# ukrbublik/You-Can-Not-Recommend

Hardware: AMD Instinct MI355X
Metric: ALS ratings/sec per iteration (U+I solve) (higher is better)
Workload: dtype f32

## Files before the change

you-can-not-recommend_amd/csrc/als_kernels.hip.h:

```cpp
#pragma once
#include <hip/hip_runtime.h>
#include <type_traits>
#include <stdint.h>
#include "schedule.h"

#ifndef YCNR_FUSED_WAVES_PER_SIMD
#define YCNR_FUSED_WAVES_PER_SIMD 2
#endif
#ifndef YCNR_FUSED_PREFETCH
#define YCNR_FUSED_PREFETCH 2
#endif

#ifndef YCNR_DUAL_BATCH
#define YCNR_DUAL_BATCH true
#endif
#ifndef YCNR_SLAB_PREFETCH
#define YCNR_SLAB_PREFETCH 3
#endif
#ifndef YCNR_DPP_PIVOTS
#define YCNR_DPP_PIVOTS 1
#endif
#ifndef YCNR_EDGE4_SOLVE
#define YCNR_EDGE4_SOLVE 1
#endif
// ... 2376 lines not shown
  const bool remF32 = krem == 4 || krem == 8;
  const int ksteps32 = remF32 ? (k >> 5) : ((k + 31) >> 5);
  const int first = 4 * (int)blockIdx.x;
  Unit us[4];
#pragma unroll
  for (int s = 0; s < 4; ++s) us[s] = a.units[a.firstDual + min(first + s, count - 1)];
  int ns[4];
#pragma unroll
  for (int s = 0; s < 4; ++s) ns[s] = (int)(us[s].end - us[s].beg);
  const int nmax = max(max(ns[0], ns[1]), max(ns[2], ns[3]));
  const int n_g = g == 0 ? ns[0] : g == 1 ? ns[1] : g == 2 ? ns[2] : ns[3];
  const int64_t beg_g = g == 0 ? us[0].beg : g == 1 ? us[1].beg : g == 2 ? us[2].beg : us[3].beg;
  const int row_g = g == 0 ? us[0].row : g == 1 ? us[1].row : g == 2 ? us[2].row : us[3].row;
  const bool valid_g = first + g < count;
  const int64_t q_g = beg_g + (c < n_g ? c : n_g - 1);
  const unsigned id_g = (unsigned)a.indx[q_g];
  float y = c < n_g ? a.vals[q_g] : 0.0f;
  acc_t acc[4];
#pragma unroll
  for (int s = 0; s < 4; ++s) {
    const int64_t q = us[s].beg + (c < ns[s] ? c : ns[s] - 1);
    const float *rowp = c < ns[s] ? a.fixed + (int64_t)a.indx[q] * k : a.zeros;
    float4 z[KS][2];
#pragma unroll
    for (int kk = 0; kk < KS; ++kk) {
      const int f = 32 * kk + 8 * g;
      z[kk][0] = *reinterpret_cast<const float4 *>(f < k ? rowp + f : a.zeros);
      z[kk][1] = *reinterpret_cast<const float4 *>(f + 4 < k ? rowp + f + 4 : a.zeros);
    }
    acc_t t = acc_t{0.0f, 0.0f, 0.0f, 0.0f};
    if (remF32) {
      const float y0 = rowp[(k & ~31) + g];
      t = Tr::mma(y0, y0, t);
      if (krem == 8) {
        const float y1 = rowp[(k & ~31) + 4 + g];
        t = Tr::mma(y1, y1, t);
      }
    }
#pragma unroll
    for (int kk = 0; kk < KS; ++kk) {
      if (kk < ksteps32) {
        const float x[8] = {z[kk][0].x, z[kk][0].y, z[kk][0].z, z[kk][0].w, z[kk][1].x, z[kk][1].y, z[kk][1].z, z[kk][1].w};
        unsigned h[4], m[4], l[4];
#pragma unroll
        for (int jj = 0; jj < 4; ++jj) {
          const float x0 = x[2 * jj], x1 = x[2 * jj + 1];
          const unsigned u0 = __builtin_bit_cast(unsigned, x0), u1 = __builtin_bit_cast(unsigned, x1);
          h[jj] = __builtin_amdgcn_perm(u1, u0, 0x07060302);
          const float s0 = x0 - __builtin_bit_cast(float, u0 & 0xFFFF0000u);
          const float s1 = x1 - __builtin_bit_cast(float, u1 & 0xFFFF0000u);
          const unsigned v0 = __builtin_bit_cast(unsigned, s0), v1 = __builtin_bit_cast(unsigned, s1);
          m[jj] = __builtin_amdgcn_perm(v1, v0, 0x07060302);
          const float t0 = s0 - __builtin_bit_cast(float, v0 & 0xFFFF0000u);
          const float t1 = s1 - __builtin_bit_cast(float, v1 & 0xFFFF0000u);
          l[jj] = __builtin_amdgcn_perm(__builtin_bit_cast(unsigned, t1), __builtin_bit_cast(unsigned, t0), 0x07060302);
        }
        const bf16x8 p1 = __builtin_bit_cast(bf16x8, u32x4{h[0], h[1], h[2], h[3]});
        const bf16x8 p2 = __builtin_bit_cast(bf16x8, u32x4{m[0], m[1], m[2], m[3]});
        const bf16x8 p3 = __builtin_bit_cast(bf16x8, u32x4{l[0], l[1], l[2], l[3]});
        t = __builtin_amdgcn_mfma_f32_16x16x32_bf16(p2, p2, t, 0, 0, 0);
        t = __builtin_amdgcn_mfma_f32_16x16x32_bf16(p1, p3, t, 0, 0, 0);
        t = __builtin_amdgcn_mfma_f32_16x16x32_bf16(p3, p1, t, 0, 0, 0);
        t = __builtin_amdgcn_mfma_f32_16x16x32_bf16(p1, p2, t, 0, 0, 0);
        t = __builtin_amdgcn_mfma_f32_16x16x32_bf16(p2, p1, t, 0, 0, 0);
        t = __builtin_amdgcn_mfma_f32_16x16x32_bf16(p1, p1, t, 0, 0, 0);
      }
    }
    acc[s] = t;
  }
  float R[16];
#pragma unroll
  for (int t = 0; t < 4; ++t) {
    const acc_t in = acc_t{acc[0][t], acc[1][t], acc[2][t], acc[3][t]};
    float out[4];
    Sv::transpose_rg(in, out);
#pragma unroll
    for (int q = 0; q < 4; ++q) R[4 * q + t] = out[q];
  }
  {
    const float dv = c < n_g ? (float)(a.lambda * (double)n_g) : 1.0f;
#pragma unroll
    for (int m = 0; m < 16; ++m) R[m] += c == m ? dv : 0.0f;
  }
  float myinv = 1.0f;
  bool bad = false;
  auto bc = [](float v, auto P) { return Sv::template row_bcast<decltype(P)::value>(v); };
  auto pivot = [&](auto P) {
    constexpr int p = decltype(P)::value;
    const float d = bc(R[p], P);
    bad = bad || !(d > 0.0f);
    const float inv = __builtin_amdgcn_rcpf(d);
    const float m = c > p ? R[p] * inv : 0.0f;
    myinv = c == p ? inv : myinv;
    auto upd = [&](auto J) {
      constexpr int j = decltype(J)::value;
      if constexpr (j > p) R[j] = fmaf(-m, bc(R[j], P), R[j]);
    };
    upd(std::integral_constant<int, 1>{}); upd(std::integral_constant<int, 2>{}); upd(std::integral_constant<int, 3>{});
    upd(std::integral_constant<int, 4>{}); upd(std::integral_constant<int, 5>{}); upd(std::integral_constant<int, 6>{});
    upd(std::integral_constant<int, 7>{}); upd(std::integral_constant<int, 8>{}); upd(std::integral_constant<int, 9>{});
    upd(std::integral_constant<int, 10>{}); upd(std::integral_constant<int, 11>{}); upd(std::integral_constant<int, 12>{});
    upd(std::integral_constant<int, 13>{}); upd(std::integral_constant<int, 14>{}); upd(std::integral_constant<int, 15>{});
    y = fmaf(-m, bc(y, P), y);
  };
#define YCNR_P(N) pivot(std::integral_constant<int, N>{});
  YCNR_P(0) YCNR_P(1) YCNR_P(2) YCNR_P(3) YCNR_P(4) YCNR_P(5) YCNR_P(6) YCNR_P(7)
  YCNR_P(8) YCNR_P(9) YCNR_P(10) YCNR_P(11) YCNR_P(12) YCNR_P(13) YCNR_P(14) YCNR_P(15)
#undef YCNR_P
  float w = 0.0f;
  auto back = [&](auto J) {
    constexpr int j = decltype(J)::value;
    const float t = y * myinv;
    w = c == j ? t : w;
    y = fmaf(-R[j], bc(t, J), y);
  };
#define YCNR_B(N) back(std::integral_constant<int, N>{});
  YCNR_B(15) YCNR_B(14) YCNR_B(13) YCNR_B(12) YCNR_B(11) YCNR_B(10) YCNR_B(9) YCNR_B(8)
  YCNR_B(7) YCNR_B(6) YCNR_B(5) YCNR_B(4) YCNR_B(3) YCNR_B(2) YCNR_B(1) YCNR_B(0)
#undef YCNR_B
  const char *base = reinterpret_cast<const char *>(a.fixed);
  const unsigned off0 = (unsigned)min(c, kq - 1) * 16u, off1 = (unsigned)min(c + 16, kq - 1) * 16u;
  float4 x0 = float4{0.0f, 0.0f, 0.0f, 0.0f}, x1 = float4{0.0f, 0.0f, 0.0f, 0.0f};
  auto gather = [&](auto I) {
    constexpr int i = decltype(I)::value;
    if (i < nmax) {
      const unsigned idi = __builtin_bit_cast(unsigned, bc(__builtin_bit_cast(float, id_g), I));
      const float wi = bc(w, I);
      const unsigned ro = idi * (unsigned)(k * 4);
      const float4 v0 = *reinterpret_cast<const float4 *>(base + (ro + off0));
      const float4 v1 = *reinterpret_cast<const float4 *>(base + (ro + off1));
      x0.x = fmaf(v0.x, wi, x0.x); x0.y = fmaf(v0.y, wi, x0.y); x0.z = fmaf(v0.z, wi, x0.z); x0.w = fmaf(v0.w, wi, x0.w);
      x1.x = fmaf(v1.x, wi, x1.x); x1.y = fmaf(v1.y, wi, x1.y); x1.z = fmaf(v1.z, wi, x1.z); x1.w = fmaf(v1.w, wi, x1.w);
    }
  };
#define YCNR_G(N) gather(std::integral_constant<int, N>{});
  YCNR_G(0) YCNR_G(1) YCNR_G(2) YCNR_G(3) YCNR_G(4) YCNR_G(5) YCNR_G(6) YCNR_G(7)
  YCNR_G(8) YCNR_G(9) YCNR_G(10) YCNR_G(11) YCNR_G(12) YCNR_G(13) YCNR_G(14) YCNR_G(15)
#undef YCNR_G
  if (valid_g) {
    float *out = a.solved + (int64_t)row_g * k;
    if (c < kq) *reinterpret_cast<float4 *>(out + 4 * c) = x0;
    if (c + 16 < kq) *reinterpret_cast<float4 *>(out + 4 * (c + 16)) = x1;
  }
  {
    const float chk = (x0.x + x0.y + x0.z + x0.w + x1.x + x1.y + x1.z + x1.w) * 0.0f;
    const unsigned long long m = __ballot(valid_g && (bad || !(chk == 0.0f)));
    if (c == 0 && ((m >> (16 * g)) & 0xFFFFull)) {
      atomicAdd(&a.err->count, 1);
      a.err->firstRow = row_g;
    }
  }
}

template <typename T, int NB, bool LDS_SOLVER, bool E4, bool FEW>
constexpr int reduce_waves() {
  if (!FEW || sizeof(T) != 4 || LDS_SOLVER) return 1;
  return NB <= 6 ? 3 : NB == 7 ? (E4 ? 3 : 2) : 1;
}
template <typename T, int NB, bool LDS_SOLVER, bool EDGE, bool E4 = false, bool FEW = false>
__global__ __launch_bounds__(64, (reduce_waves<T, NB, LDS_SOLVER, E4, FEW>())) void als_reduce_solve_kernel(StepArgs<T> a) {
  extern __shared__ __attribute__((aligned(16))) unsigned char smem[];
  using G = typename GramSel<T, NB, EDGE>::type;
  using acc_t = typename G::acc_t;
  const int lane = threadIdx.x;
  const SplitRow sr = a.split[blockIdx.x];
  typename G::State st;
  G::init(st);
  bool wide = false;
  if constexpr (std::is_same<T, float>::value && !FEW) wide = sr.nslabs > kFewSlabs;
  if (wide) {
    if constexpr (std::is_same<T, float>::value && !FEW)
      G::sum_slabs_wide(st, a.slabs + (int64_t)sr.slab0 * (G::slab_regs() * 64) + lane, sr.nslabs);
  } else {
    for (int sl = 0; sl < sr.nslabs; ++sl) G::add_slab(st, a.slabs + (int64_t)(sr.slab0 + sl) * (G::slab_regs() * 64) + lane);
  }
  acc_t acc[G::NT];
  T bacc[NB];
  G::to_tiles(st, acc, bacc, reinterpret_cast<T *>(smem), lane);
  const T lam = (T)(a.lambda * (double)sr.n);
  if constexpr (E4 && std::is_same<T, float>::value && !LDS_SOLVER) {
    SolveMfmaF32<NB>::template run<true>(acc, bacc, reinterpret_cast<float *>(smem), a.k, lam, a.solved + (int64_t)sr.row * a.k, sr.row, a.err, lane,
                                         a.kReal > 0 ? a.kReal : -1);
  } else {
    SolverFor<T, NB, LDS_SOLVER>::type::run(acc, bacc, reinterpret_cast<T *>(smem), a.k, lam,
                                          a.solved + (int64_t)sr.row * a.k, sr.row, a.err, lane, a.kReal > 0 ? a.kReal : -1);
  }
}


template <typename T>
__global__ __launch_bounds__(256) void als_slab_sum_kernel(T *arena, const SlabSum *list, int64_t elems) {
  const SlabSum e = list[blockIdx.x];
  for (int64_t i = threadIdx.x; i < elems; i += 256) {
    const T *src = arena + e.src0 + i;
    if (std::is_same<T, float>::value && e.n > kFewSlabs) {
      double v = 0.0;
      for (int s = 0; s < e.n; ++s) v += (double)src[(int64_t)s * elems];
      arena[e.dst + i] = (T)v;
    } else {
      T v = T(0);
      for (int s = 0; s < e.n; ++s) v += src[(int64_t)s * elems];
      arena[e.dst + i] = v;
    }
  }
}

template <typename T, int NB, bool LDS_SOLVER, bool EDGE, bool E4 = false>
__global__ __launch_bounds__(64, 1) void als_band_reduce_solve_kernel(StepArgs<T> a, const T *const *bandSlab, int32_t nBands) {
  extern __shared__ __attribute__((aligned(16))) unsigned char smem[];
  using G = typename GramSel<T, NB, EDGE>::type;
  using acc_t = typename G::acc_t;
  const int lane = threadIdx.x;
  const SplitRow sr = a.split[blockIdx.x];
  typename G::State st;
  G::init(st);
  for (int b = 0; b < nBands; ++b) {
    const T *p = bandSlab[(int64_t)sr.slab0 + b];
    if (p) G::add_slab(st, p + lane);
  }
  acc_t acc[G::NT];
  T bacc[NB];
  G::to_tiles(st, acc, bacc, reinterpret_cast<T *>(smem), lane);
  const T lam = (T)(a.lambda * (double)sr.n);
  if constexpr (E4 && std::is_same<T, float>::value && !LDS_SOLVER) {
    SolveMfmaF32<NB>::template run<true>(acc, bacc, reinterpret_cast<float *>(smem), a.k, lam, a.solved + (int64_t)sr.row * a.k, sr.row, a.err, lane,
                                         a.kReal > 0 ? a.kReal : -1);
  } else {
    SolverFor<T, NB, LDS_SOLVER>::type::run(acc, bacc, reinterpret_cast<T *>(smem), a.k, lam,
                                          a.solved + (int64_t)sr.row * a.k, sr.row, a.err, lane, a.kReal > 0 ? a.kReal : -1);
  }
}

template <typename T>
struct RmseArgs {
  const int64_t *rowPtr;
  const int32_t *indx;
  const T *vals;
  const T *userFactors;
  const T *itemFactors;
  const int64_t *portionRowEnd;
  double *out;
  double shift;
  int64_t rowBegin;
  int32_t k;
};

#ifndef YCNR_RMSE_RB
#define YCNR_RMSE_RB 4
#endif
template <typename T, int NCH>
__global__ __launch_bounds__(256) void als_rmse_kernel(RmseArgs<T> a) {
  __shared__ double red[3][16];
  const int tid = threadIdx.x, grp = tid >> 4, l16 = tid & 15;
  const int p = blockIdx.x;
  const int64_t r0 = p == 0 ? 0 : a.portionRowEnd[p - 1];
  const int64_t r1 = a.portionRowEnd[p];
  double sd2 = 0, sp = 0, cnt = 0;
  typedef T vec4 __attribute__((ext_vector_type(4)));
  constexpr int NC = NCH > 0 ? NCH : 1;
  constexpr int RB = NCH == 0 ? 1 : (NCH * (int)sizeof(T) <= 8 ? YCNR_RMSE_RB : (NCH * (int)sizeof(T) <= 16 ? YCNR_RMSE_RB / 2 : YCNR_RMSE_RB / 4));
  const int nchunk = a.k >> 2;
  for (int64_t r = r0 + grp; r < r1; r += 16) {
    const T *uF = a.userFactors + (a.rowBegin + r) * a.k;
    vec4 u[NC];
    if constexpr (NCH > 0) {
#pragma unroll
      for (int i = 0; i < NCH; ++i) {
        const int ch = l16 + 16 * i;
        u[i] = ch < nchunk ? *reinterpret_cast<const vec4 *>(uF + 4 * ch) : vec4{T(0), T(0), T(0), T(0)};
      }
    }
    const int64_t q1 = a.rowPtr[r + 1];
    for (int64_t q = a.rowPtr[r]; q < q1; q += RB) {
      int32_t id[RB];
      T val[RB];
#pragma unroll
      for (int j = 0; j < RB; ++j) {
        const int64_t qq = q + j < q1 ? q + j : q1 - 1;
        id[j] = a.indx[qq];
        val[j] = a.vals[qq];
      }
      vec4 v[RB][NC];
      if constexpr (NCH > 0) {
#pragma unroll
        for (int j = 0; j < RB; ++j) {
          const T *iF = a.itemFactors + (int64_t)id[j] * a.k;
#pragma unroll
          for (int i = 0; i < NCH; ++i) {
            const int ch = l16 + 16 * i;
            v[j][i] = ch < nchunk ? *reinterpret_cast<const vec4 *>(iF + 4 * ch) : vec4{T(0), T(0), T(0), T(0)};
          }
        }
      }
#pragma unroll
      for (int j = 0; j < RB; ++j) {
        T dot = T(0);
        if constexpr (NCH > 0) {
#pragma unroll
          for (int i = 0; i < NCH; ++i) {
            dot = fma(u[i][0], v[j][i][0], dot);
            dot = fma(u[i][1], v[j][i][1], dot);
            dot = fma(u[i][2], v[j][i][2], dot);
            dot = fma(u[i][3], v[j][i][3], dot);
          }
        } else {
          const T *iF = a.itemFactors + (int64_t)id[j] * a.k;
// ... 55 lines not shown
```

you-can-not-recommend_amd/csrc/kernel_choice.h:

```cpp
#pragma once

#ifndef YCNR_EDGE4_SOLVE
#define YCNR_EDGE4_SOLVE 1
#endif

namespace ycnr {

enum GramForm { kGramMfma, kGramX6, kGramX6D, kGramPlanes };

struct KernelChoice {
  int nb;
  bool ldsSolver;
  GramForm chunk;
  bool chunkEdge, chunkPadRhs, chunkPk3;
  GramForm row;
  bool rowEdge, rowE4, rowPadRhs, rowPk3, rowPack;
  bool reduceEdge, reduceE4, reduceFew, bandE4;
  bool rowLdsImage;
};

inline KernelChoice choose_kernels(bool f64, int k, bool ldsSolver, bool edge, bool x6, bool hasPlanes, bool fewSlabs, bool noX6d,
                                   bool noFusedX6d, bool noPk3) {
  const int nb = (k + 15) / 16;
  KernelChoice c = {};
  c.nb = nb, c.ldsSolver = ldsSolver, c.rowLdsImage = true;
  if (f64) return c;
  edge = edge && nb >= 2;
  const bool first4 = k == 16 * (nb - 1) + 4;
  const bool padRhs = k < 16 * nb;
  const bool e4 = YCNR_EDGE4_SOLVE && nb >= 2 && !ldsSolver && first4;
  const bool x6d = x6 && k % 4 == 0 && !noX6d;
  const bool pk3 = padRhs && first4 && !noPk3;
  c.chunk = x6d ? kGramX6D : x6 ? kGramX6 : kGramMfma;
  c.chunkEdge = c.reduceEdge = edge && !x6;
  c.chunkPadRhs = x6d && padRhs;
  c.chunkPk3 = x6d && pk3;
  c.reduceE4 = c.bandE4 = e4;
  c.reduceFew = fewSlabs && !ldsSolver;
  if (x6 && hasPlanes && !ldsSolver && k % 4 == 0 && padRhs) {
    c.row = kGramPlanes;
    c.rowPack = c.rowE4 = nb >= 2 && first4;
    c.rowLdsImage = false;
  } else if (x6d && !noFusedX6d && !(ldsSolver && nb == 8)) {
    c.row = kGramX6D;
    c.rowPadRhs = padRhs;
    c.rowE4 = e4;
    c.rowPk3 = pk3;
  } else {
    c.row = kGramMfma;
    c.rowEdge = edge;
    c.rowE4 = e4;
  }
  return c;
}

}
```

you-can-not-recommend_amd/csrc/ycnr_als.hip:

```cpp
#include "../../include/ycnr_als.h"
#include "als_kernels.hip.h"
#include "kernel_choice.h"
#include "als_wg_kernels.hip.h"
#include "als_pair_kernels.hip.h"
#ifdef YCNR_WITH_G32
#include "devtest/als_gram32_kernels.hip.h"
#endif
#include "als_gen_kernels.hip.h"
#include "prep_kernels.hip.h"
#include <hipcub/hipcub.hpp>
#include "recommend_kernels.hip.h"

#include <algorithm>
#include <cfloat>
#include <cstdarg>
#include <cstdio>
#include <cstdlib>
#include <cmath>
#include <cstring>
#include <functional>
#include <map>
#include <mutex>
#include <new>
#include <string>
#include <type_traits>
#include <vector>

using namespace ycnr;

namespace {

thread_local std::string g_last_error;

int fail(int code, const char *fmt, ...) {
  char buf[1024];
  va_list ap;
  va_start(ap, fmt);
  vsnprintf(buf, sizeof buf, fmt, ap);
  va_end(ap);
  g_last_error = buf;
  return code;
}

#define HIP_TRY(expr)                                                                           \
  do {                                                                                          \
    hipError_t e_ = (expr);                                                                     \
    if (e_ != hipSuccess)                                                                       \
      return fail(e_ == hipErrorOutOfMemory ? YCNR_ERR_NOMEM : YCNR_ERR_HIP, "%s failed: %s (%s:%d)", \
                  #expr, hipGetErrorString(e_), __FILE__, __LINE__);                            \
  } while (0)

constexpr int kMaxFactors = 128;
constexpr int kMaxFactorsBig = 256;
constexpr int kMaxFactorsAny = 4096;
constexpr int64_t kGenArenaBytes = (int64_t)2 << 30;
constexpr int kPairNB = 16;
constexpr int64_t kPairBatchRows = 4096;
constexpr int64_t kBandBytes = (int64_t)96 << 20;
constexpr size_t kErrBytes = 65536;
constexpr size_t kZeroRowBytes = 32768 + 64;
constexpr int kMaxDualBlocksSmallK = 5;

size_t tsize(int dtype) { return dtype == YCNR_F64 ? 8 : 4; }

struct Ratings {
  int64_t rowBegin = 0, rowEnd = 0, nnz = 0;
  int64_t *dRowPtr = nullptr;
  int32_t *dIndx = nullptr;
  void *dVals = nullptr;
  bool loaded = false;
  void release() {
    if (dRowPtr) (void)hipFree(dRowPtr);
    if (dIndx) (void)hipFree(dIndx);
    if (dVals) (void)hipFree(dVals);
    dRowPtr = nullptr;
    dIndx = nullptr;
    dVals = nullptr;
    loaded = false;
    nnz = 0;
  }
};


bool is_gen(int dtype, int k) { return k > (dtype == YCNR_F32 ? kMaxFactorsBig : kMaxFactors); }

struct Schedule : PlanCounts {
  std::vector<GenBatch> genBatches;
  Unit *dUnits = nullptr;
  SplitRow *dSplit = nullptr;
  void *dSlabs = nullptr;
  float *dRowSlabs = nullptr;
  int64_t rowSlabRows = 0;
  int64_t nUnits = 0, nSplit = 0;
  void release() {
    if (dUnits) (void)hipFree(dUnits);
    if (dSplit) (void)hipFree(dSplit);
    if (dSlabs) (void)hipFree(dSlabs);
    if (dRowSlabs) (void)hipFree(dRowSlabs);
    *this = Schedule();
  }
};

struct EnvFlags {
  bool noDualX6, noX6d, noFusedX6d, noOverlap, ignoreNumeric, noDualQuad, noGraph, noPair, g32, noPk3;
  size_t k1LdsPad;
};
const EnvFlags &env_flags() {
  static const EnvFlags f = {getenv("YCNR_NO_DUAL_X6") != nullptr, getenv("YCNR_NO_X6D") != nullptr, getenv("YCNR_NO_FUSED_X6D") != nullptr,
                             getenv("YCNR_NO_OVERLAP") != nullptr, getenv("YCNR_IGNORE_NUMERIC") != nullptr, getenv("YCNR_NO_DUAL_QUAD") != nullptr,
                             getenv("YCNR_NO_GRAPH") != nullptr, getenv("YCNR_NO_PAIR") != nullptr, getenv("YCNR_G32") != nullptr, getenv("YCNR_NO_PK3") != nullptr,
                             getenv("YCNR_K1_LDSPAD") ? (size_t)atoi(getenv("YCNR_K1_LDSPAD")) : 0};
  return f;
}

int set_max_lds(const void *fn, size_t bytes) {
  static std::mutex mu;
  static std::map<std::pair<const void *, int>, size_t> done;
  int dev = 0;
  HIP_TRY(hipGetDevice(&dev));
  std::lock_guard<std::mutex> lock(mu);
  auto it = done.find({fn, dev});
  if (it != done.end() && it->second == bytes) return YCNR_OK;
  HIP_TRY(hipFuncSetAttribute(fn, hipFuncAttributeMaxDynamicSharedMemorySize, (int)bytes));
  done[{fn, dev}] = bytes;
  return YCNR_OK;
}

constexpr int kSideStreams = 6;
int g_hw_queues_at_load = 0;
__attribute__((constructor)) void ycnr_note_hw_queues() {
  const char *q = getenv("GPU_MAX_HW_QUEUES");
  g_hw_queues_at_load = q ? atoi(q) : 0;
}
int side_streams() {
  static const int n = [] {
    const char *e = getenv("YCNR_SIDE_STREAMS");
    if (e) return std::max(1, std::min(kSideStreams, atoi(e)));
    return g_hw_queues_at_load >= 8 ? 5 : 2;
  }();
  return n;
}
constexpr int64_t kGraphMaxRatings = 2 * 1024 * 1024;
constexpr int64_t kGraphMinRatings = 256 * 1024;
constexpr int64_t kMinOverlapDualRows = 1024;

struct DualPlan {
  bool noX6 = false;
  bool fewSlabs = false;
  int64_t nPrimal = -1;
  const int64_t *first = nullptr, *count = nullptr;
  int nSide = 0;
  hipStream_t side[kSideStreams] = {};
  hipEvent_t fork = nullptr, join[kSideStreams] = {};
  mutable int nextSide = 0;
  hipStream_t slabStream = nullptr;
  hipEvent_t slabJoin = nullptr;
};

template <int M>
int launch_dual(StepArgs<float> args, const DualPlan &dp, hipStream_t stream) {
  if (dp.count[M] > 0) {
    if (dp.nSide > 0) stream = dp.side[dp.nextSide++ % dp.nSide];
    args.firstDual = (int32_t)dp.first[M];
    if constexpr (M == 1) {
      if (!dp.noX6 && !env_flags().noDualX6 && !env_flags().noDualQuad && args.k <= 128 && args.k % 4 == 0 && args.fixedBytes != 0) {
        hipLaunchKernelGGL(als_dual_quad_kernel, dim3((unsigned)((dp.count[M] + 3) / 4)), dim3(64), 0, stream, args, (int32_t)dp.count[M]);
        HIP_TRY(hipGetLastError());
        return YCNR_OK;
      }
    }
    const bool x6 = !dp.noX6 && !env_flags().noDualX6;
    void (*kd)(StepArgs<float>) = als_dual_solve_kernel<M, false>;
    if (x6) kd = als_dual_solve_kernel<M, true>;
    static const size_t ldsPad = getenv("YCNR_DUAL_LDSPAD") ? (size_t)atoi(getenv("YCNR_DUAL_LDSPAD")) : 0;
    if (ldsPad)
      if (int rcl = set_max_lds(reinterpret_cast<const void *>(kd), SolveMfmaF32<M>::lds_bytes() + ldsPad)) return rcl;
    hipLaunchKernelGGL(kd, dim3((unsigned)dp.count[M]), dim3(64), SolveMfmaF32<M>::lds_bytes() + ldsPad, stream, args);
    HIP_TRY(hipGetLastError());
  }
  return YCNR_OK;
}

template <typename T>
void launch_rmse(const RmseArgs<T> &a, int nPieces, hipStream_t stream) {
  const bool vec = ((size_t)a.k * sizeof(T)) % 16 == 0 && a.k <= 512;
  void (*kr)(RmseArgs<T>) = als_rmse_kernel<T, 0>;
  if (vec) kr = a.k <= 64 ? als_rmse_kernel<T, 1> : a.k <= 128 ? als_rmse_kernel<T, 2> : a.k <= 256 ? als_rmse_kernel<T, 4> : als_rmse_kernel<T, 8>;
  hipLaunchKernelGGL(kr, dim3((unsigned)nPieces), dim3(256), 0, stream, a);
}

template <typename T, int M = kMaxDualBlocks>
int launch_duals(const StepArgs<T> &args, const DualPlan &dp, hipStream_t stream) {
  if constexpr (std::is_same<T, float>::value && M > 0) {
    if (int rc = launch_dual<M>(args, dp, stream)) return rc;
    return launch_duals<T, M - 1>(args, dp, stream);
  }
  return YCNR_OK;
}

template <typename T>
int fork_duals(const StepArgs<T> &args, const DualPlan &dp, hipStream_t stream) {
  for (int i = 0; i < dp.nSide; ++i) HIP_TRY(hipStreamWaitEvent(dp.side[i], dp.fork, 0));
  dp.nextSide = 0;
  if (int rc = launch_duals<T>(args, dp, stream)) return rc;
  for (int i = 0; i < dp.nSide; ++i) HIP_TRY(hipEventRecord(dp.join[i], dp.side[i]));
  return YCNR_OK;
}
int join_duals(const DualPlan &dp, hipStream_t stream) {
  for (int i = 0; i < dp.nSide; ++i) HIP_TRY(hipStreamWaitEvent(stream, dp.join[i], 0));
  return YCNR_OK;
}

template <bool CAN, typename F>
auto with_bool(bool b, F f) {
  if constexpr (CAN)
    if (b) return f(std::true_type());
  return f(std::false_type());
}
template <int LO, int HI, typename F>
bool dispatch_nb(int nb, F &&f) {
  if constexpr (LO <= HI) return nb == LO ? (f(std::integral_constant<int, LO>()), true) : dispatch_nb<LO + 1, HI>(nb, f);
  else return false;
}

template <typename T>
struct RowKernels {
  void (*chunk)(StepArgs<T>), (*row)(StepArgs<T>), (*reduce)(StepArgs<T>);
  void (*band)(StepArgs<T>, const T *const *, int32_t);
  size_t ldsRow, ldsReduce;
};

template <typename T, int NB, bool LDSV>
void row_kernels_nb(const KernelChoice &c, RowKernels<T> &r) {
  constexpr bool F32 = std::is_same<T, float>::value, EDGE = F32 && NB >= 2, E4 = EDGE && !LDSV;
  using Fn = void (*)(StepArgs<T>);
  r.ldsReduce = SolverFor<T, NB, LDSV>::type::lds_bytes();
  r.ldsRow = c.rowLdsImage ? r.ldsReduce : 0;
  if (c.chunk == kGramMfma) r.chunk = with_bool<EDGE>(c.chunkEdge, [](auto e) -> Fn { return als_gram_slab_kernel<T, NB, decltype(e)::value>; });
  if (c.row == kGramMfma)
    r.row = with_bool<EDGE>(c.rowEdge, [&](auto e) { return with_bool<E4>(c.rowE4, [](auto e4) -> Fn { return als_gram_solve_kernel<T, NB, LDSV, decltype(e)::value, decltype(e4)::value>; }); });
  if constexpr (F32) {
    if (c.chunk == kGramX6) r.chunk = als_gram_slab_x6_kernel<NB>;
    if (c.chunk == kGramX6D)
      r.chunk = !c.chunkPadRhs ? als_gram_slab_x6d_kernel<NB, false> : c.chunkPk3 ? als_gram_slab_x6d_kernel<NB, true, true> : als_gram_slab_x6d_kernel<NB, true, false>;
    if constexpr (!(LDSV && NB == 8))
      if (c.row == kGramX6D)
        r.row = !c.rowPadRhs ? als_gram_solve_x6d_kernel<NB, false, LDSV, false> : with_bool<E4>(c.rowE4, [&](auto e4) -> Fn {
          return c.rowPk3 ? als_gram_solve_x6d_kernel<NB, true, LDSV, decltype(e4)::value, true> : als_gram_solve_x6d_kernel<NB, true, LDSV, decltype(e4)::value, false>;
        });
    if constexpr (!LDSV)
      if (c.row == kGramPlanes) r.row = with_bool<EDGE>(c.rowPack, [](auto p) -> Fn { return als_gram_solve_x6p_kernel<NB, decltype(p)::value, decltype(p)::value>; });
  }
  r.reduce = with_bool<EDGE>(c.reduceEdge, [&](auto e) { return with_bool<E4>(c.reduceE4, [&](auto e4) {
    return with_bool<F32 && !LDSV>(c.reduceFew, [](auto few) -> Fn { return als_reduce_solve_kernel<T, NB, LDSV, decltype(e)::value, decltype(e4)::value, decltype(few)::value>; });
  }); });
  r.band = with_bool<EDGE>(c.reduceEdge, [&](auto e) { return with_bool<E4>(c.bandE4, [](auto e4) -> decltype(r.band) { return als_band_reduce_solve_kernel<T, NB, LDSV, decltype(e)::value, decltype(e4)::value>; }); });
}

template <typename T>
int row_kernels(const StepArgs<T> &args, bool ldsSolver, bool edge, bool x6, bool fewSlabs, RowKernels<T> &r) {
  const KernelChoice c = choose_kernels(std::is_same<T, double>::value, args.k, ldsSolver, edge, x6, args.planes != nullptr, fewSlabs,
                                        env_flags().noX6d, env_flags().noFusedX6d, env_flags().noPk3);
  r = RowKernels<T>{};
  if (!dispatch_nb<1, 8>(c.nb, [&](auto nb) { ldsSolver ? row_kernels_nb<T, decltype(nb)::value, true>(c, r) : row_kernels_nb<T, decltype(nb)::value, false>(c, r); }))
    return fail(YCNR_ERR_UNSUPPORTED, "factorsCount %d > %d is not supported by this build", args.k, kMaxFactors);
  if (!r.chunk || !r.row || !r.reduce || !r.band) return fail(YCNR_ERR_UNSUPPORTED, "factorsCount %d: no kernel of the chosen form in this build", args.k);
  return YCNR_OK;
}

template <typename T>
int launch_rows(const RowKernels<T> &rk, StepArgs<T> args, int64_t nUnits, int64_t nSplitUnits, int64_t nSplit, hipStream_t stream,
                hipEvent_t *ev , const DualPlan &dp) {
  const size_t lds = rk.ldsReduce, ldsRow = rk.ldsRow + env_flags().k1LdsPad;
  if (int rcl = set_max_lds(reinterpret_cast<const void *>(rk.row), ldsRow)) return rcl;
  if (int rcl = set_max_lds(reinterpret_cast<const void *>(rk.reduce), lds)) return rcl;
  args.firstFused = (int32_t)nSplitUnits;
  if (ev) HIP_TRY(hipEventRecord(ev[0], stream));
  const bool branch = dp.slabStream != nullptr && nSplitUnits > 0;
  const int64_t nPrimal = dp.nPrimal >= 0 ? dp.nPrimal : nUnits - nSplitUnits;
  const bool overlap = dp.nPrimal >= 0 && dp.nSide > 0;
  if (branch || overlap) HIP_TRY(hipEventRecord(dp.fork, stream));
  if (branch) {
    HIP_TRY(hipStreamWaitEvent(dp.slabStream, dp.fork, 0));
    hipLaunchKernelGGL(rk.chunk, dim3((unsigned)nSplitUnits), dim3(64), 0, dp.slabStream, args);
    HIP_TRY(hipGetLastError());
    if (nSplit > 0) {
      hipLaunchKernelGGL(rk.reduce, dim3((unsigned)nSplit), dim3(64), lds, dp.slabStream, args);
      HIP_TRY(hipGetLastError());
    }
    HIP_TRY(hipEventRecord(dp.slabJoin, dp.slabStream));
  } else if (nSplitUnits > 0) {
    hipLaunchKernelGGL(rk.chunk, dim3((unsigned)nSplitUnits), dim3(64), 0, stream, args);
    HIP_TRY(hipGetLastError());
  }
  if (ev) HIP_TRY(hipEventRecord(ev[1], stream));
  if (overlap)
    if (int rc = fork_duals<T>(args, dp, stream)) return rc;
  if (nPrimal > 0) {
    hipLaunchKernelGGL(rk.row, dim3((unsigned)nPrimal), dim3(64), ldsRow, stream, args);
    HIP_TRY(hipGetLastError());
  }
  if (ev) HIP_TRY(hipEventRecord(ev[2], stream));
  if (int rc = overlap ? join_duals(dp, stream) : dp.nPrimal >= 0 ? launch_duals<T>(args, dp, stream) : YCNR_OK) return rc;
  if (ev) HIP_TRY(hipEventRecord(ev[3], stream));
  if (branch) {
    HIP_TRY(hipStreamWaitEvent(stream, dp.slabJoin, 0));
  } else if (nSplit > 0) {
    hipLaunchKernelGGL(rk.reduce, dim3((unsigned)nSplit), dim3(64), lds, stream, args);
    HIP_TRY(hipGetLastError());
  }
  if (ev) HIP_TRY(hipEventRecord(ev[4], stream));
  return YCNR_OK;
}

__global__ void pad_rows_kernel(const float *src, float *dst, int64_t rowBegin, int64_t rows, int k, int kp) {
  const int64_t i = (int64_t)blockIdx.x * blockDim.x + threadIdx.x;
  if (i >= rows * kp) return;
  const int64_t r = rowBegin + i / kp;
  const int c = (int)(i % kp);
  dst[r * kp + c] = c < k ? src[r * k + c] : 0.0f;
}
__global__ void unpad_rows_kernel(const float *src, float *dst, int64_t rowBegin, int64_t rows, int k, int kp) {
  const int64_t i = (int64_t)blockIdx.x * blockDim.x + threadIdx.x;
  if (i >= rows * k) return;
  const int64_t r = rowBegin + i / k;
  const int c = (int)(i % k);
// ... 2552 lines not shown
```

Before: 5.934 billion.

## Add four-rows-per-wave dual solve kernel for 17-32 rating rows

Adds a kernel that handles four small (2-block, up to 32 ratings) dual-form rows per 64-lane wave. It builds the 32x32 Gram with split-bf16 MFMAs and a small LDS transpose, then runs a register-resident DPP Cholesky-style elimination and a gather back-projection. The goal is to cut per-row launch and occupancy waste from the one-row-per-block dual solve for M=2. It adds a selection helper with an env opt-out and a fixedBytes<4GiB guard for 32-bit offsets. It also brings more register pressure and numerics that depend on the bf16x3 split.

```diff
diff --git a/you-can-not-recommend_amd/csrc/als_kernels.hip.h b/you-can-not-recommend_amd/csrc/als_kernels.hip.h
--- a/you-can-not-recommend_amd/csrc/als_kernels.hip.h
+++ b/you-can-not-recommend_amd/csrc/als_kernels.hip.h
@@ -2552,6 +2552,256 @@
   }
 }
 
+__global__ __launch_bounds__(64, 2) void als_dual_quad2_kernel(StepArgs<float> a, int32_t count) {
+  using Sv = SolveMfmaF32<1>;
+  using Tr = MfmaTraits<float>;
+  using acc_t = typename Tr::acc_t;
+  typedef __bf16 bf16x8 __attribute__((ext_vector_type(8)));
+  typedef unsigned u32x4 __attribute__((ext_vector_type(4)));
+  constexpr int KS = 4;
+  constexpr int LDW = 20;
+  __shared__ __attribute__((aligned(16))) float ldsT01[4 * 16 * LDW];
+  const int lane = threadIdx.x, g = lane >> 4, c = lane & 15;
+  const int k = a.k, kq = k >> 2;
+  const int krem = k & 31;
+  const bool remF32 = krem == 4 || krem == 8;
+  const int ksteps32 = remF32 ? (k >> 5) : ((k + 31) >> 5);
+  const int first = 4 * (int)blockIdx.x;
+  Unit us[4];
+#pragma unroll
+  for (int s = 0; s < 4; ++s) us[s] = a.units[a.firstDual + min(first + s, count - 1)];
+  int ns[4];
+#pragma unroll
+  for (int s = 0; s < 4; ++s) ns[s] = (int)(us[s].end - us[s].beg);
+  const int nmax = max(max(ns[0], ns[1]), max(ns[2], ns[3]));
+  const int n_g = g == 0 ? ns[0] : g == 1 ? ns[1] : g == 2 ? ns[2] : ns[3];
+  const int64_t beg_g = g == 0 ? us[0].beg : g == 1 ? us[1].beg : g == 2 ? us[2].beg : us[3].beg;
+  const int row_g = g == 0 ? us[0].row : g == 1 ? us[1].row : g == 2 ? us[2].row : us[3].row;
+  const bool valid_g = first + g < count;
+  const int64_t qA = beg_g + (c < n_g ? c : n_g - 1), qB = beg_g + (c + 16 < n_g ? c + 16 : n_g - 1);
+  const unsigned idA = (unsigned)a.indx[qA], idB = (unsigned)a.indx[qB];
+  float yA = c < n_g ? a.vals[qA] : 0.0f, yB = c + 16 < n_g ? a.vals[qB] : 0.0f;
+  acc_t acc[4][3];
+  auto split8 = [](const float4 &z0, const float4 &z1, bf16x8 &o1, bf16x8 &o2, bf16x8 &o3) {
+    const float x[8] = {z0.x, z0.y, z0.z, z0.w, z1.x, z1.y, z1.z, z1.w};
+    unsigned h[4], m[4], l[4];
+#pragma unroll
+    for (int jj = 0; jj < 4; ++jj) {
+      const float x0 = x[2 * jj], x1 = x[2 * jj + 1];
+      const unsigned u0 = __builtin_bit_cast(unsigned, x0), u1 = __builtin_bit_cast(unsigned, x1);
+      h[jj] = __builtin_amdgcn_perm(u1, u0, 0x07060302);
+      const float s0 = x0 - __builtin_bit_cast(float, u0 & 0xFFFF0000u);
+      const float s1 = x1 - __builtin_bit_cast(float, u1 & 0xFFFF0000u);
+      const unsigned v0 = __builtin_bit_cast(unsigned, s0), v1 = __builtin_bit_cast(unsigned, s1);
+      m[jj] = __builtin_amdgcn_perm(v1, v0, 0x07060302);
+      const float t0 = s0 - __builtin_bit_cast(float, v0 & 0xFFFF0000u);
+      const float t1 = s1 - __builtin_bit_cast(float, v1 & 0xFFFF0000u);
+      l[jj] = __builtin_amdgcn_perm(__builtin_bit_cast(unsigned, t1), __builtin_bit_cast(unsigned, t0), 0x07060302);
+    }
+    o1 = __builtin_bit_cast(bf16x8, u32x4{h[0], h[1], h[2], h[3]});
+    o2 = __builtin_bit_cast(bf16x8, u32x4{m[0], m[1], m[2], m[3]});
+    o3 = __builtin_bit_cast(bf16x8, u32x4{l[0], l[1], l[2], l[3]});
+  };
+#pragma unroll
+  for (int s = 0; s < 4; ++s) {
+    const float *rowp[2];
+#pragma unroll
+    for (int b = 0; b < 2; ++b) {
+      const int i = 16 * b + c;
+      const int64_t q = us[s].beg + (i < ns[s] ? i : ns[s] - 1);
+      rowp[b] = i < ns[s] ? a.fixed + (int64_t)a.indx[q] * k : a.zeros;
+    }
+    float4 z[2][KS][2];
+#pragma unroll
+    for (int kk = 0; kk < KS; ++kk) {
+      const int f = 32 * kk + 8 * g;
+#pragma unroll
+      for (int b = 0; b < 2; ++b) {
+        z[b][kk][0] = *reinterpret_cast<const float4 *>(f < k ? rowp[b] + f : a.zeros);
+        z[b][kk][1] = *reinterpret_cast<const float4 *>(f + 4 < k ? rowp[b] + f + 4 : a.zeros);
+      }
+    }
+    acc_t t00 = acc_t{0.0f, 0.0f, 0.0f, 0.0f}, t01 = t00, t11 = t00;
+    if (remF32) {
+      const float a0 = rowp[0][(k & ~31) + g], b0 = rowp[1][(k & ~31) + g];
+      t00 = Tr::mma(a0, a0, t00);
+      t01 = Tr::mma(a0, b0, t01);
+      t11 = Tr::mma(b0, b0, t11);
+      if (krem == 8) {
+        const float a1 = rowp[0][(k & ~31) + 4 + g], b1 = rowp[1][(k & ~31) + 4 + g];
+        t00 = Tr::mma(a1, a1, t00);
+        t01 = Tr::mma(a1, b1, t01);
+        t11 = Tr::mma(b1, b1, t11);
+      }
+    }
+#pragma unroll
+    for (int kk = 0; kk < KS; ++kk) {
+      if (kk < ksteps32) {
+        bf16x8 a1, a2, a3, b1, b2, b3;
+        split8(z[0][kk][0], z[0][kk][1], a1, a2, a3);
+        split8(z[1][kk][0], z[1][kk][1], b1, b2, b3);
+#define YCNR_T3(A0, A1, B0, B1)                                              \
+  t00 = __builtin_amdgcn_mfma_f32_16x16x32_bf16(A0, A1, t00, 0, 0, 0);       \
+  t01 = __builtin_amdgcn_mfma_f32_16x16x32_bf16(A0, B1, t01, 0, 0, 0);       \
+  t11 = __builtin_amdgcn_mfma_f32_16x16x32_bf16(B0, B1, t11, 0, 0, 0);
+        YCNR_T3(a2, a2, b2, b2)
+        YCNR_T3(a1, a3, b1, b3)
+        YCNR_T3(a3, a1, b3, b1)
+        YCNR_T3(a1, a2, b1, b2)
+        YCNR_T3(a2, a1, b2, b1)
+        YCNR_T3(a1, a1, b1, b1)
+#undef YCNR_T3
+      }
+    }
+    acc[s][0] = t00, acc[s][1] = t01, acc[s][2] = t11;
+#pragma unroll
+    for (int t = 0; t < 4; ++t) ldsT01[(16 * s + 4 * g + t) * LDW + c] = t01[t];
+  }
+  float RA[32], RB[32];
+#pragma unroll
+  for (int X = 0; X < 3; ++X) {
+#pragma unroll
+    for (int t = 0; t < 4; ++t) {
+      const acc_t in = acc_t{acc[0][X][t], acc[1][X][t], acc[2][X][t], acc[3][X][t]};
+      float out[4];
+      Sv::transpose_rg(in, out);
+#pragma unroll
+      for (int q = 0; q < 4; ++q) {
+        if (X == 0) RA[4 * q + t] = out[q];
+        if (X == 1) RB[4 * q + t] = out[q];
+        if (X == 2) RB[16 + 4 * q + t] = out[q];
+      }
+    }
+  }
+  __syncthreads();
+#pragma unroll
+  for (int q = 0; q < 4; ++q) {
+    const float4 v = *reinterpret_cast<const float4 *>(&ldsT01[(16 * g + c) * LDW + 4 * q]);
+    RA[16 + 4 * q] = v.x, RA[16 + 4 * q + 1] = v.y, RA[16 + 4 * q + 2] = v.z, RA[16 + 4 * q + 3] = v.w;
+  }
+  {
+    const float lam = (float)(a.lambda * (double)n_g);
+    const float dA = c < n_g ? lam : 1.0f, dB = c + 16 < n_g ? lam : 1.0f;
+#pragma unroll
+    for (int m = 0; m < 16; ++m) {
+      RA[m] += c == m ? dA : 0.0f;
+      RB[16 + m] += c == m ? dB : 0.0f;
+    }
+  }
+  float invA = 1.0f, invB = 1.0f;
+  bool bad = false;
+  auto bc = [](float v, auto P) { return Sv::template row_bcast<decltype(P)::value>(v); };
+  auto pivotA = [&](auto P) {
+    constexpr int p = decltype(P)::value;
+    const float d = bc(RA[p], P);
+    bad = bad || !(d > 0.0f);
+    const float inv = __builtin_amdgcn_rcpf(d);
+    const float mA = c > p ? -(RA[p] * inv) : 0.0f;
+    const float mB = -(RB[p] * inv);
+    invA = c == p ? inv : invA;
+#pragma unroll
+    for (int j = p + 1; j < 32; ++j) {
+      if (j == p + 1)
+        asm("s_nop 1\n\tv_fmac_f32_dpp %0, %1, %2 row_newbcast:%3 row_mask:0xf bank_mask:0xf bound_ctrl:1" : "+v"(RB[j]) : "v"(RA[j]), "v"(mB), "n"(p));
+      else
+        asm("v_fmac_f32_dpp %0, %1, %2 row_newbcast:%3 row_mask:0xf bank_mask:0xf bound_ctrl:1" : "+v"(RB[j]) : "v"(RA[j]), "v"(mB), "n"(p));
+      if (j == 31)
+        asm("v_fmac_f32_dpp %0, %0, %1 row_newbcast:%2 row_mask:0xf bank_mask:0xf bound_ctrl:1\n\ts_nop 1" : "+v"(RA[j]) : "v"(mA), "n"(p));
+      else
+        asm("v_fmac_f32_dpp %0, %0, %1 row_newbcast:%2 row_mask:0xf bank_mask:0xf bound_ctrl:1" : "+v"(RA[j]) : "v"(mA), "n"(p));
+    }
+    const float r = bc(yA, P);
+    yA = fmaf(r, mA, yA);
+    yB = fmaf(r, mB, yB);
+  };
+  auto pivotB = [&](auto P) {
+    constexpr int p = decltype(P)::value;
+    const float d = bc(RB[16 + p], P);
+    bad = bad || !(d > 0.0f);
+    const float inv = __builtin_amdgcn_rcpf(d);
+    const float m = c > p ? -(RB[16 + p] * inv) : 0.0f;
+    invB = c == p ? inv : invB;
+#pragma unroll
+    for (int j = 16 + p + 1; j < 32; ++j) {
+      if (j == 16 + p + 1 && j == 31)
+        asm("s_nop 1\n\tv_fmac_f32_dpp %0, %0, %1 row_newbcast:%2 row_mask:0xf bank_mask:0xf bound_ctrl:1\n\ts_nop 1" : "+v"(RB[j]) : "v"(m), "n"(p));
+      else if (j == 16 + p + 1)
+        asm("s_nop 1\n\tv_fmac_f32_dpp %0, %0, %1 row_newbcast:%2 row_mask:0xf bank_mask:0xf bound_ctrl:1" : "+v"(RB[j]) : "v"(m), "n"(p));
+      else if (j == 31)
+        asm("v_fmac_f32_dpp %0, %0, %1 row_newbcast:%2 row_mask:0xf bank_mask:0xf bound_ctrl:1\n\ts_nop 1" : "+v"(RB[j]) : "v"(m), "n"(p));
+      else
+        asm("v_fmac_f32_dpp %0, %0, %1 row_newbcast:%2 row_mask:0xf bank_mask:0xf bound_ctrl:1" : "+v"(RB[j]) : "v"(m), "n"(p));
+    }
+    yB = fmaf(bc(yB, P), m, yB);
+  };
+#define YCNR_P(N) pivotA(std::integral_constant<int, N>{});
+  YCNR_P(0) YCNR_P(1) YCNR_P(2) YCNR_P(3) YCNR_P(4) YCNR_P(5) YCNR_P(6) YCNR_P(7)
+  YCNR_P(8) YCNR_P(9) YCNR_P(10) YCNR_P(11) YCNR_P(12) YCNR_P(13) YCNR_P(14) YCNR_P(15)
+#undef YCNR_P
+#define YCNR_P(N) pivotB(std::integral_constant<int, N>{});
+  YCNR_P(0) YCNR_P(1) YCNR_P(2) YCNR_P(3) YCNR_P(4) YCNR_P(5) YCNR_P(6) YCNR_P(7)
+  YCNR_P(8) YCNR_P(9) YCNR_P(10) YCNR_P(11) YCNR_P(12) YCNR_P(13) YCNR_P(14) YCNR_P(15)
+#undef YCNR_P
+  float wA = 0.0f, wB = 0.0f;
+  auto backB = [&](auto J) {
+    constexpr int j = decltype(J)::value;
+    const float t = yB * invB;
+    wB = c == j ? t : wB;
+    const float tb = bc(t, J);
+    yB = fmaf(-RB[16 + j], tb, yB);
+    yA = fmaf(-RA[16 + j], tb, yA);
+  };
+  auto backA = [&](auto J) {
+    constexpr int j = decltype(J)::value;
+    const float t = yA * invA;
+    wA = c == j ? t : wA;
+    yA = fmaf(-RA[j], bc(t, J), yA);
+  };
+#define YCNR_B(N) backB(std::integral_constant<int, N>{});
+  YCNR_B(15) YCNR_B(14) YCNR_B(13) YCNR_B(12) YCNR_B(11) YCNR_B(10) YCNR_B(9) YCNR_B(8)
+  YCNR_B(7) YCNR_B(6) YCNR_B(5) YCNR_B(4) YCNR_B(3) YCNR_B(2) YCNR_B(1) YCNR_B(0)
+#undef YCNR_B
+#define YCNR_B(N) backA(std::integral_constant<int, N>{});
+  YCNR_B(15) YCNR_B(14) YCNR_B(13) YCNR_B(12) YCNR_B(11) YCNR_B(10) YCNR_B(9) YCNR_B(8)
+  YCNR_B(7) YCNR_B(6) YCNR_B(5) YCNR_B(4) YCNR_B(3) YCNR_B(2) YCNR_B(1) YCNR_B(0)
+#undef YCNR_B
+  const char *base = reinterpret_cast<const char *>(a.fixed);
+  const unsigned off0 = (unsigned)min(c, kq - 1) * 16u, off1 = (unsigned)min(c + 16, kq - 1) * 16u;
+  float4 x0 = float4{0.0f, 0.0f, 0.0f, 0.0f}, x1 = float4{0.0f, 0.0f, 0.0f, 0.0f};
+  auto gather = [&](auto I, unsigned id, float w, int i) {
+    if (i < nmax) {
+      const unsigned idi = __builtin_bit_cast(unsigned, bc(__builtin_bit_cast(float, id), I));
+      const float wi = bc(w, I);
+      const unsigned ro = idi * (unsigned)(k * 4);
+      const float4 v0 = *reinterpret_cast<const float4 *>(base + (ro + off0));
+      const float4 v1 = *reinterpret_cast<const float4 *>(base + (ro + off1));
+      x0.x = fmaf(v0.x, wi, x0.x); x0.y = fmaf(v0.y, wi, x0.y); x0.z = fmaf(v0.z, wi, x0.z); x0.w = fmaf(v0.w, wi, x0.w);
+      x1.x = fmaf(v1.x, wi, x1.x); x1.y = fmaf(v1.y, wi, x1.y); x1.z = fmaf(v1.z, wi, x1.z); x1.w = fmaf(v1.w, wi, x1.w);
+    }
+  };
+#define YCNR_G(N) gather(std::integral_constant<int, N>{}, idA, wA, N);
+  YCNR_G(0) YCNR_G(1) YCNR_G(2) YCNR_G(3) YCNR_G(4) YCNR_G(5) YCNR_G(6) YCNR_G(7)
+  YCNR_G(8) YCNR_G(9) YCNR_G(10) YCNR_G(11) YCNR_G(12) YCNR_G(13) YCNR_G(14) YCNR_G(15)
+#undef YCNR_G
+#define YCNR_G(N) gather(std::integral_constant<int, N>{}, idB, wB, 16 + N);
+  YCNR_G(0) YCNR_G(1) YCNR_G(2) YCNR_G(3) YCNR_G(4) YCNR_G(5) YCNR_G(6) YCNR_G(7)
+  YCNR_G(8) YCNR_G(9) YCNR_G(10) YCNR_G(11) YCNR_G(12) YCNR_G(13) YCNR_G(14) YCNR_G(15)
+#undef YCNR_G
+  if (valid_g) {
+    float *out = a.solved + (int64_t)row_g * k;
+    if (c < kq) *reinterpret_cast<float4 *>(out + 4 * c) = x0;
+    if (c + 16 < kq) *reinterpret_cast<float4 *>(out + 4 * (c + 16)) = x1;
+  }
+  {
+    const float chk = (x0.x + x0.y + x0.z + x0.w + x1.x + x1.y + x1.z + x1.w) * 0.0f;
+    const unsigned long long m = __ballot(valid_g && (bad || !(chk == 0.0f)));
+    if (c == 0 && ((m >> (16 * g)) & 0xFFFFull)) {
+      atomicAdd(&a.err->count, 1);
+      a.err->firstRow = row_g;
+    }
+  }
+}
+
 template <typename T, int NB, bool LDS_SOLVER, bool E4, bool FEW>
 constexpr int reduce_waves() {
   if (!FEW || sizeof(T) != 4 || LDS_SOLVER) return 1;
diff --git a/you-can-not-recommend_amd/csrc/kernel_choice.h b/you-can-not-recommend_amd/csrc/kernel_choice.h
--- a/you-can-not-recommend_amd/csrc/kernel_choice.h
+++ b/you-can-not-recommend_amd/csrc/kernel_choice.h
@@ -54,4 +54,15 @@
   return c;
 }
 
+enum DualForm { kDualSolve, kDualSolveX6, kDualQuad, kDualQuad2 };
+
+inline DualForm choose_dual(int blocks, int k, unsigned long long fixedBytes, bool noBf16x6, bool noDualX6, bool noDualQuad,
+                            bool noDualQuad2) {
+  if (noBf16x6 || noDualX6) return kDualSolve;
+  const bool fourRows = k <= 128 && k % 4 == 0 && fixedBytes != 0 && fixedBytes < (1ull << 32);
+  if (blocks == 1 && fourRows && !noDualQuad) return kDualQuad;
+  if (blocks == 2 && fourRows && !noDualQuad2) return kDualQuad2;
+  return kDualSolveX6;
 }
+
+}
diff --git a/you-can-not-recommend_amd/csrc/ycnr_als.hip b/you-can-not-recommend_amd/csrc/ycnr_als.hip
--- a/you-can-not-recommend_amd/csrc/ycnr_als.hip
+++ b/you-can-not-recommend_amd/csrc/ycnr_als.hip
@@ -102,13 +102,13 @@
 };
 
 struct EnvFlags {
-  bool noDualX6, noX6d, noFusedX6d, noOverlap, ignoreNumeric, noDualQuad, noGraph, noPair, g32, noPk3;
+  bool noDualX6, noX6d, noFusedX6d, noOverlap, ignoreNumeric, noDualQuad, noDualQuad2, noGraph, noPair, g32, noPk3;
   size_t k1LdsPad;
 };
 const EnvFlags &env_flags() {
   static const EnvFlags f = {getenv("YCNR_NO_DUAL_X6") != nullptr, getenv("YCNR_NO_X6D") != nullptr, getenv("YCNR_NO_FUSED_X6D") != nullptr,
                              getenv("YCNR_NO_OVERLAP") != nullptr, getenv("YCNR_IGNORE_NUMERIC") != nullptr, getenv("YCNR_NO_DUAL_QUAD") != nullptr,
-                             getenv("YCNR_NO_GRAPH") != nullptr, getenv("YCNR_NO_PAIR") != nullptr, getenv("YCNR_G32") != nullptr, getenv("YCNR_NO_PK3") != nullptr,
+                             getenv("YCNR_NO_DUAL_QUAD2") != nullptr, getenv("YCNR_NO_GRAPH") != nullptr, getenv("YCNR_NO_PAIR") != nullptr, getenv("YCNR_G32") != nullptr, getenv("YCNR_NO_PK3") != nullptr,
                              getenv("YCNR_K1_LDSPAD") ? (size_t)atoi(getenv("YCNR_K1_LDSPAD")) : 0};
   return f;
 }
@@ -162,16 +162,15 @@
   if (dp.count[M] > 0) {
     if (dp.nSide > 0) stream = dp.side[dp.nextSide++ % dp.nSide];
     args.firstDual = (int32_t)dp.first[M];
-    if constexpr (M == 1) {
-      if (!dp.noX6 && !env_flags().noDualX6 && !env_flags().noDualQuad && args.k <= 128 && args.k % 4 == 0 && args.fixedBytes != 0) {
-        hipLaunchKernelGGL(als_dual_quad_kernel, dim3((unsigned)((dp.count[M] + 3) / 4)), dim3(64), 0, stream, args, (int32_t)dp.count[M]);
-        HIP_TRY(hipGetLastError());
-        return YCNR_OK;
-      }
-    }
-    const bool x6 = !dp.noX6 && !env_flags().noDualX6;
+    const DualForm form = choose_dual(M, args.k, args.fixedBytes, dp.noX6, env_flags().noDualX6, env_flags().noDualQuad, env_flags().noDualQuad2);
+    if (form == kDualQuad || form == kDualQuad2) {
+      void (*kq)(StepArgs<float>, int32_t) = form == kDualQuad ? als_dual_quad_kernel : als_dual_quad2_kernel;
+      hipLaunchKernelGGL(kq, dim3((unsigned)((dp.count[M] + 3) / 4)), dim3(64), 0, stream, args, (int32_t)dp.count[M]);
+      HIP_TRY(hipGetLastError());
+      return YCNR_OK;
+    }
     void (*kd)(StepArgs<float>) = als_dual_solve_kernel<M, false>;
-    if (x6) kd = als_dual_solve_kernel<M, true>;
+    if (form == kDualSolveX6) kd = als_dual_solve_kernel<M, true>;
     static const size_t ldsPad = getenv("YCNR_DUAL_LDSPAD") ? (size_t)atoi(getenv("YCNR_DUAL_LDSPAD")) : 0;
     if (ldsPad)
       if (int rcl = set_max_lds(reinterpret_cast<const void *>(kd), SolveMfmaF32<M>::lds_bytes() + ldsPad)) return rcl;
```

After: 5.931 billion. No clear change (-0.1%).
